# Rose-STL-Lab/spherical-dyffusion

Hardware: AMD Instinct MI355X
Metric: forecast-steps/sec (180x360, 63ch), 25-member ensemble DYffusion sampling, whole job (higher is better)
Workload: dtype f32 tensors; every GEMM-class kernel (1x1 convs, fused MLP, Legendre analysis/synthesis, dhconv) as 3-pass split-f16 MFMA with f32 accumulation; FFT / norms / pointwise in f32 (statistics f64); 1 GPU; 25-member ensemble x horizon-6 DYffusion sampling pass (6 forecaster + 10 interpolator SFNO forwards, dropout stream on, AR feedback), 180x360, 63 state + 2 forcing channels, embed 256, 8 blocks; horizon=6, relayed_members=0, parallelism=members of one initial condition sharded over GPUs, no data-path collective

## Files before the change

### spherical-dyffusion_amd/csrc/fft360.hip

```cpp
#include "common.h"
#include "fft.h"

namespace {

typedef float c2 __attribute__((ext_vector_type(2)));

constexpr int NH = 180;
constexpr int NLON = 360;
constexpr int ROWS = 16;
constexpr int NT = 256;
constexpr int P = 200;
constexpr int Q4 = NLON / 4;
constexpr int MIT = 3;
#ifndef SDY_FFT_MINB_F
#define SDY_FFT_MINB_F 4
#endif
#ifndef SDY_FFT_MINB_I
#define SDY_FFT_MINB_I 4
#endif
#ifndef SDY_FFT_KPW
#define SDY_FFT_KPW 1
#endif
constexpr int MINB_F = SDY_FFT_MINB_F, MINB_I = SDY_FFT_MINB_I;

template <int SG>
__device__ __forceinline__ c2 mul_i(c2 a) {
  return SG > 0 ? c2{-a.y, a.x} : c2{a.y, -a.x};
}
__device__ __forceinline__ c2 cmul(c2 a, c2 w) { return a.xx * w + a.yy * c2{-w.y, w.x}; }
__device__ __forceinline__ c2 cmul_conj(c2 a, c2 w) { return a.xx * c2{w.x, -w.y} + a.yy * c2{w.y, w.x}; }

template <int SG>
__device__ __forceinline__ void dft3(c2& v0, c2& v1, c2& v2) {
  const float sn = 0.86602540378443864676f;
  const c2 a = v1 + v2, b = v1 - v2;
  const c2 m = v0 - 0.5f * a;
  const c2 t = mul_i<SG>(sn * b);
  v0 = v0 + a;
  v1 = m + t;
  v2 = m - t;
}
template <int SG>
__device__ __forceinline__ void dft4(c2& v0, c2& v1, c2& v2, c2& v3) {
  const c2 t0 = v0 + v2, t1 = v0 - v2, t2 = v1 + v3, t3 = mul_i<SG>(v1 - v3);
  v0 = t0 + t2;
  v1 = t1 + t3;
  v2 = t0 - t2;
  v3 = t1 - t3;
}
template <int SG>
__device__ __forceinline__ void dft5(c2& v0, c2& v1, c2& v2, c2& v3, c2& v4) {
  const float c1 = 0.30901699437494742410f, c2_ = -0.80901699437494742410f;
  const float s1 = 0.95105651629515357212f, s2 = 0.58778525229247312917f;
  const c2 a1 = v1 + v4, a2 = v2 + v3, b1 = v1 - v4, b2 = v2 - v3;
  const c2 r1 = v0 + c1 * a1 + c2_ * a2;
  const c2 r2 = v0 + c2_ * a1 + c1 * a2;
  const c2 i1 = mul_i<SG>(s1 * b1 + s2 * b2);
  const c2 i2 = mul_i<SG>(s2 * b1 - s1 * b2);
  v0 = v0 + a1 + a2;
  v1 = r1 + i1;
  v4 = r1 - i1;
  v2 = r2 + i2;
  v3 = r2 - i2;
}
template <int R, int SG>
__device__ __forceinline__ void dft_small(c2* t) {
  if constexpr (R == 3) dft3<SG>(t[0], t[1], t[2]);
  if constexpr (R == 4) dft4<SG>(t[0], t[1], t[2], t[3]);
  if constexpr (R == 5) dft5<SG>(t[0], t[1], t[2], t[3], t[4]);
}

template <int N1, int N2>
__host__ __device__ constexpr int pfa_slot(int k) { return (N2 * (k % N1) + N1 * (k % N2)) % (N1 * N2); }
template <int N1, int N2, int SG>
__device__ __forceinline__ void pfa(c2* v) {
  constexpr int N = N1 * N2;
#pragma unroll
  for (int n2 = 0; n2 < N2; ++n2) {
    c2 t[N1];
#pragma unroll
    for (int n1 = 0; n1 < N1; ++n1) t[n1] = v[(N2 * n1 + N1 * n2) % N];
    dft_small<N1, SG>(t);
#pragma unroll
    for (int n1 = 0; n1 < N1; ++n1) v[(N2 * n1 + N1 * n2) % N] = t[n1];
  }
#pragma unroll
  for (int k1 = 0; k1 < N1; ++k1) {
    c2 u[N2];
#pragma unroll
    for (int n2 = 0; n2 < N2; ++n2) u[n2] = v[(N2 * k1 + N1 * n2) % N];
    dft_small<N2, SG>(u);
#pragma unroll
    for (int n2 = 0; n2 < N2; ++n2) v[(N2 * k1 + N1 * n2) % N] = u[n2];
  }
}

struct Lane {
  int wave, lane, t;
  c2* row;
};
__device__ __forceinline__ Lane lane_roles(c2* Z) {
  Lane L;
  L.wave = __builtin_amdgcn_readfirstlane(threadIdx.x >> 6);
  L.lane = threadIdx.x & 63;
  L.t = L.lane & 15;
  const int rl = L.lane >> 4;
  L.row = Z + (4 * L.wave + (rl & 1) * 2 + (rl >> 1)) * P;
  return L;
}

constexpr int TWN = 12 * 16;
__device__ __forceinline__ void fill_twiddles(const SdyFftDesc& f, c2* TW) {
  if (threadIdx.x < TWN) {
    const int k1 = threadIdx.x >> 4, a = threadIdx.x & 15;
    TW[threadIdx.x] = reinterpret_cast<const c2*>(f.tw)[a < 15 ? a * k1 : 0];
  }
}

template <int SG, bool NYQ_COPY>
__device__ __forceinline__ void pass_b(const Lane& L) {
  __builtin_amdgcn_wave_barrier();
  if (L.t < 12) {
    c2 u[15];
    const c2* src = L.row + 15 * L.t;
#pragma unroll
    for (int a = 0; a < 15; ++a) u[a] = src[a];
    pfa<3, 5, SG>(u);
    __builtin_amdgcn_wave_barrier();
    c2* dst = L.row + L.t;
#pragma unroll
    for (int k2 = 0; k2 < 15; ++k2) dst[12 * k2] = u[pfa_slot<3, 5>(k2)];
    if (NYQ_COPY && L.t == 0) dst[NH] = u[pfa_slot<3, 5>(0)];
  }
  __builtin_amdgcn_wave_barrier();
}
template <int SG>
__device__ __forceinline__ void pass_a_tail(const Lane& L, c2* v, const c2* TW) {
  pfa<3, 4, SG>(v);
  c2* dst = L.row + L.t;
  const c2* tw = TW + L.t;
  dst[0] = v[pfa_slot<3, 4>(0)];
#pragma unroll
  for (int k1 = 1; k1 < 12; ++k1) {
    const c2 y = v[pfa_slot<3, 4>(k1)];
    dst[15 * k1] = SG < 0 ? cmul(y, tw[16 * k1]) : cmul_conj(y, tw[16 * k1]);
  }
}

constexpr int TAIL = Q4 - 64;

#ifndef SDY_FFT_GROUP
#define SDY_FFT_GROUP 4
#endif
struct WgId {
  int x, y, z;
};
__device__ __forceinline__ WgId wg_id(int nx, int ny) {
  const unsigned total = gridDim.x, L = blockIdx.x;
  const unsigned xcd = L % 8u, slot = L / 8u;
  const unsigned id = xcd * (total / 8u) + min(xcd, total % 8u) + slot;
  WgId w;
#if SDY_FFT_GROUP > 0
  if (nx % SDY_FFT_GROUP == 0) {
    const unsigned G = SDY_FFT_GROUP;
    w.x = (int)(G * ((id / (G * ny)) % ((unsigned)nx / G)) + id % G);
    w.y = (int)((id / G) % (unsigned)ny);
    w.z = (int)(id / ((unsigned)nx * ny));
    return w;
  }
#endif
  w.x = id % nx;
  w.y = (id / nx) % ny;
  w.z = id / (nx * ny);
  return w;
}

template <int KPW>
__global__ __launch_bounds__(NT, MINB_F) void rfft360_kernel(const SdyFftDesc f, const float* __restrict__ x,
                                                           const float* __restrict__ pa, const float* __restrict__ pd,
                                                           float* __restrict__ xn_out, float* __restrict__ Xf, int B,
                                                           int C, int K, int mtr, int ilv,
                                                           const int* __restrict__ mcut, const SdyImgMap xmap,
                                                           unsigned* flags, unsigned* head, int x_mod) {
  __shared__ __attribute__((aligned(16))) c2 Z[ROWS * P];
  __shared__ c2 TW[TWN];
  __shared__ c2 AD[ROWS];
  const Lane L = lane_roles(Z);
  const WgId id = wg_id(C / ROWS, (K + KPW - 1) / KPW);
  const int c0 = id.x * ROWS, b = id.z;
  const int bx = sdy_img(xmap, b);
  const int k_begin = id.y * KPW, k_end = min(K, k_begin + KPW);

  fill_twiddles(f, TW);
  if (threadIdx.x < ROWS) {
    const int s = threadIdx.x, ch = c0 + 4 * (s & 3) + (s >> 2);
    AD[s] = pa ? c2{pa[bx * C + ch], pd[bx * C + ch]} : c2{1.0f, 0.0f};
  }

  const int bsrc = x_mod > 0 ? bx % x_mod : bx;
  const float* xw = x + (((long)bsrc * C + c0 + L.wave) * K) * NLON + 4 * L.lane;
  float* xnw = xn_out ? xn_out + (((long)bx * C + c0 + L.wave) * K) * NLON + 4 * L.lane : nullptr;
  const long rstride = 4L * K * NLON;
  c2* zw = Z + 4 * L.wave * P + 2 * L.lane;
  const bool tail = L.lane < TAIL;

  const int c4 = threadIdx.x & 3, mg = threadIdx.x >> 2;
  const float scale = 6.28318530717958647692f / (float)NLON;
  c2 W[MIT];
#pragma unroll
  for (int it = 0; it < MIT; ++it) {
    const c2 w = reinterpret_cast<const c2*>(f.pw)[min(mg + 64 * it, NH)];
    W[it] = c2{w.y, -w.x} * (0.5f * scale);
  }
  const c2* za = Z + c4 * P + mg;
  const c2* zn01 = Z + c4 * P + (NH - 64 - mg);
  const c2* zn2 = Z + c4 * P + max(NH - 128 - mg, 0);
  const long mstride = (long)K * B * 2 * C;
  const int re_off = (ilv ? 2 * c0 : c0) + 4 * c4, im_off = ilv ? 16 : C;
  const long tile_base = (long)((b * (C / ROWS) + id.x) >> 1) * K * 64 + (id.x & 1) * 32 + 4 * c4;

  float amax = 0.0f;
  f32x4 regs[8];
  auto gload = [&](int k) {
#pragma unroll
    for (int r = 0; r < 4; ++r) {
      const float* src = xw + r * rstride + (long)k * NLON;
      regs[2 * r] = *reinterpret_cast<const f32x4*>(src);
      if (tail) regs[2 * r + 1] = *reinterpret_cast<const f32x4*>(src + 256);
    }
  };
  gload(k_begin);
  __syncthreads();

  for (int k = k_begin; k < k_end; ++k) {
#pragma unroll
    for (int r = 0; r < 4; ++r) {
      const c2 ad = AD[4 * L.wave + r];
      const f32x4 v0 = regs[2 * r] * ad.x + ad.y, v1 = regs[2 * r + 1] * ad.x + ad.y;
      if (xnw) {
        float* dst = xnw + r * rstride + (long)k * NLON;
        *reinterpret_cast<f32x4*>(dst) = v0;
        if (tail) *reinterpret_cast<f32x4*>(dst + 256) = v1;
      }
      *reinterpret_cast<f32x4*>(zw + r * P) = v0;
      if (tail) *reinterpret_cast<f32x4*>(zw + r * P + 128) = v1;
    }
    if (k + 1 < k_end) gload(k + 1);
    __builtin_amdgcn_wave_barrier();

    if (L.t < 15) {
      c2 v[12];
      const c2* src = L.row + L.t;
#pragma unroll
      for (int bb = 0; bb < 12; ++bb) v[bb] = src[15 * bb];
      pass_a_tail<-1>(L, v, TW);
    }
    pass_b<-1, true>(L);
    __syncthreads();

    float* Xk = ilv == 2 ? Xf + tile_base + (long)k * 64 : Xf + ((long)k * B + b) * 2 * C + re_off;
    const int mlive = mcut ? min(mtr, mcut[k]) : mtr;
#pragma unroll
    for (int it = 0; it < MIT; ++it) {
      const int m = mg + 64 * it;
      if (m < mlive) {
        f32x4 vr, vi;
#pragma unroll
        for (int j = 0; j < 4; ++j) {
          const c2 A = za[64 * it + 4 * j * P];
          const c2 Bv = it < 2 ? zn01[64 * (1 - it) + 4 * j * P] : zn2[4 * j * P];
          const c2 S = c2{A.x + Bv.x, A.y - Bv.y}, D = c2{A.x - Bv.x, A.y + Bv.y};
          const c2 X = (0.5f * scale) * S + cmul(D, W[it]);
          vr[j] = X.x;
          vi[j] = X.y;
          amax = __builtin_fmaxf(amax, __builtin_fmaxf(__builtin_fabsf(X.x), __builtin_fabsf(X.y)));
        }
        float* o = Xk + (long)m * mstride;
        SDY_STREAM_STORE(o, vr);
        SDY_STREAM_STORE(o + im_off, vi);
      }
    }
    __syncthreads();
  }
  sdy_flag_range(flags, amax * (2.0f * SDY_ACT_SX), head);
}

template <int KPW>
__global__ __launch_bounds__(NT, MINB_I) void irfft360_kernel(const SdyFftDesc f, const float* __restrict__ Yf,
                                                            const float* __restrict__ bias, float* __restrict__ y, int B,
                                                            int C, int K, int mtr, int ilv,
                                                            const int* __restrict__ mcut, float* __restrict__ zt,
                                                            long zt_bs, double* __restrict__ part) {
  __shared__ __attribute__((aligned(16))) c2 Z[ROWS * P];
  __shared__ c2 TW[TWN];
  __shared__ c2 PW[NH];
  __shared__ float BS[ROWS];
  const Lane L = lane_roles(Z);
  const WgId id = wg_id(C / ROWS, (K + KPW - 1) / KPW);
  const int c0 = id.x * ROWS, b = id.z;
  const int k_begin = id.y * KPW, k_end = min(K, k_begin + KPW);

  fill_twiddles(f, TW);
  if (threadIdx.x < NH) {
    const c2 w = reinterpret_cast<const c2*>(f.pw)[threadIdx.x];
    PW[threadIdx.x] = c2{w.x, -w.y};
  }
  if (threadIdx.x < ROWS) {
    const int s = threadIdx.x;
    BS[s] = bias ? bias[c0 + 4 * (s & 3) + (s >> 2)] : 0.0f;
  }

  const int c4 = threadIdx.x & 3, mg = threadIdx.x >> 2;
  const long mstride = (long)K * B * 2 * C;
  const int re_off = (ilv ? 2 * c0 : c0) + 4 * c4, im_off = ilv ? 16 : C;
  const long tile_base = (long)((b * (C / ROWS) + id.x) >> 1) * K * 64 + (id.x & 1) * 32 + 4 * c4;
  f32x4 rr[MIT], ri[MIT];
  auto gload = [&](int k) {
    const float* Yk = ilv == 2 ? Yf + tile_base + (long)k * 64 : Yf + ((long)k * B + b) * 2 * C + re_off;
    const int mlive = mcut ? min(mtr, mcut[k]) : mtr;
#pragma unroll
    for (int it = 0; it < MIT; ++it) {
      const int m = mg + 64 * it;
      f32x4 vr = {0.f, 0.f, 0.f, 0.f}, vi = {0.f, 0.f, 0.f, 0.f};
      if (m < mlive) {
        const float* o = Yk + (long)m * mstride;
        vr = *reinterpret_cast<const f32x4*>(o);
        vi = *reinterpret_cast<const f32x4*>(o + im_off);
      }
      if (m == 0 || m == NH) vi = f32x4{0.f, 0.f, 0.f, 0.f};
      rr[it] = vr;
      ri[it] = vi;
    }
  };

  float* yw = y + (((long)b * C + c0 + L.wave) * K) * NLON + 4 * L.lane;
  const long rstride = 4L * K * NLON;
  const c2* zw = Z + 4 * L.wave * P + 2 * L.lane;
  const bool tail = L.lane < TAIL;
  c2* zs = Z + c4 * P + mg;

  gload(k_begin);
  for (int k = k_begin; k < k_end; ++k) {
#pragma unroll
    for (int it = 0; it < MIT; ++it) {
      if (mg + 64 * it <= NH) {
#pragma unroll
        for (int j = 0; j < 4; ++j) zs[4 * j * P + 64 * it] = c2{rr[it][j], ri[it][j]};
      }
    }
    __syncthreads();
    if (k + 1 < k_end) gload(k + 1);

    if (L.t < 15) {
      c2 v[12];
      const c2* lo = L.row + L.t;
      const c2* hi = L.row + (15 - L.t);
      const c2* pw = PW + L.t;
#pragma unroll
      for (int bb = 0; bb < 12; ++bb) {
        const c2 A = lo[15 * bb], Bv = hi[15 * (11 - bb)], w = pw[15 * bb];
        const c2 S = c2{A.x + Bv.x, A.y - Bv.y}, Dm = c2{A.x - Bv.x, A.y + Bv.y};
        const c2 D = cmul(Dm, w);
        v[bb] = c2{S.x - D.y, S.y + D.x};
      }
      __builtin_amdgcn_wave_barrier();
      pass_a_tail<+1>(L, v, TW);
    }
    pass_b<+1, false>(L);

    if (zt) {
      float* ztb = zt + (long)b * zt_bs;
      const int px0 = k * NLON + 4 * L.lane, px1 = px0 + 256;
#pragma unroll
      for (int r = 0; r < 4; ++r) {
        const float bs = BS[4 * L.wave + r];
        const int ch = c0 + L.wave + 4 * r;
        f32x4 v = *reinterpret_cast<const f32x4*>(zw + r * P) + bs;
        v = f32x4{gelu_erf(v.x), gelu_erf(v.y), gelu_erf(v.z), gelu_erf(v.w)};
        SDY_STREAM_STORE(ztb + (long)(px0 >> 6) * (C * 64) + ch * 64 + (px0 & 63), v);
        float qs = sdy_quad_sum(v), qs2 = sdy_quad_sumsq(v);
        if (tail) {
          f32x4 u = *reinterpret_cast<const f32x4*>(zw + r * P + 128) + bs;
          u = f32x4{gelu_erf(u.x), gelu_erf(u.y), gelu_erf(u.z), gelu_erf(u.w)};
          SDY_STREAM_STORE(ztb + (long)(px1 >> 6) * (C * 64) + ch * 64 + (px1 & 63), u);
          qs += sdy_quad_sum(u);
          qs2 += sdy_quad_sumsq(u);
        }
        double ds = (double)row16_sum(qs), ds2 = (double)row16_sum(qs2);
        ds += __shfl_xor(ds, 16, 64);
        ds2 += __shfl_xor(ds2, 16, 64);
        ds += __shfl_xor(ds, 32, 64);
        ds2 += __shfl_xor(ds2, 32, 64);
        if (L.lane == 0) {
          double* slot = part + (((long)b * K + k) * C + ch) * 2;
          slot[0] = ds;
          slot[1] = ds2;
        }
      }
    } else {
#pragma unroll
    for (int r = 0; r < 4; ++r) {
      const float bs = BS[4 * L.wave + r];
      float* dst = yw + r * rstride + (long)k * NLON;
      SDY_STREAM_STORE(dst, *reinterpret_cast<const f32x4*>(zw + r * P) + bs);
      if (tail) SDY_STREAM_STORE(dst + 256, *reinterpret_cast<const f32x4*>(zw + r * P + 128) + bs);
    }
    }
    __syncthreads();
  }
}

}

int sdy_fft360_launch_fwd(const SdyFftDesc& f, const float* x, const float* a, const float* d, float* xn_out, float* Xf,
                          int B, int C, int K, int mtr, int ilv, const int* mcut, hipStream_t stream,
                          const unsigned char* x_rows, int x_mod) {
  if (f.n != NH || C % ROWS != 0 || mtr > NH + 1 || (long)ROWS * K * NLON >= (1L << 31)) return SDY_ERR_UNSUPPORTED;
  if (ilv == 2 && (C % (2 * ROWS) != 0 || ROWS != 16)) return SDY_ERR_UNSUPPORTED;
  constexpr int KPW = SDY_FFT_KPW;
  SdyImgMap xmap;
  SDY_TRY(sdy_img_map_fill(xmap, x_rows, B));
  dim3 grid((C / ROWS) * ((K + KPW - 1) / KPW) * B);
  unsigned *flags = nullptr, *head = nullptr;
  if (f.guard_f16) {
    SDY_TRY(sdy_flags_ptr(&flags));
    SDY_TRY(sdy_headroom_ptr(SDY_RANGE_LEG_ANALYSIS, &head));
  }
  hipLaunchKernelGGL((rfft360_kernel<KPW>), grid, dim3(NT), 0, stream, f, x, a, d, xn_out, Xf, B, C, K, mtr, ilv, mcut, xmap,
                     flags, head, x_mod);
  return sdy_launch_status();
}

int sdy_fft360_launch_inv(const SdyFftDesc& f, const float* Yf, const float* bias, float* y, int B, int C, int K,
                          int mtr, int ilv, const int* mcut, hipStream_t stream, float* zt, long zt_bs, double* part) {
  if (f.n != NH || C % ROWS != 0 || mtr > NH + 1 || (long)ROWS * K * NLON >= (1L << 31)) return SDY_ERR_UNSUPPORTED;
  if (ilv == 2 && (C % (2 * ROWS) != 0 || ROWS != 16)) return SDY_ERR_UNSUPPORTED;
  if ((zt == nullptr) != (part == nullptr) || (!zt && !y)) return SDY_ERR_ARG;
  constexpr int KPW = SDY_FFT_KPW;
  dim3 grid((C / ROWS) * ((K + KPW - 1) / KPW) * B);
  hipLaunchKernelGGL((irfft360_kernel<KPW>), grid, dim3(NT), 0, stream, f, Yf, bias, y, B, C, K, mtr, ilv, mcut, zt, zt_bs, part);
  return sdy_launch_status();
}
```

Baseline: 165.1 member-forecast-steps/s.

## Shrink inverse FFT LDS row pitch, raise its occupancy bound, add timing stamps

Splits the shared-memory row pitch into separate forward and inverse values and cuts the inverse kernel's pitch from 200 to 184 complex elements. This lowers its LDS footprint, and with launch_bounds min blocks raised from 4 to 6 more workgroups can be resident per CU. A static_assert keeps the pitch at 8 or 24 mod 32 to avoid bank conflicts. It also adds env-gated s_memtime instrumentation and occupancy query exports under SDY_STAMPS_ON. The tighter launch bound may force register spills in the inverse kernel.

```diff
diff --git a/spherical-dyffusion_amd/csrc/fft360.hip b/spherical-dyffusion_amd/csrc/fft360.hip
--- a/spherical-dyffusion_amd/csrc/fft360.hip
+++ b/spherical-dyffusion_amd/csrc/fft360.hip
@@ -1,3 +1,5 @@
+#include <cstdlib>
+
 #include "common.h"
 #include "fft.h"
 
@@ -9,14 +11,21 @@
 constexpr int NLON = 360;
 constexpr int ROWS = 16;
 constexpr int NT = 256;
-constexpr int P = 200;
+#ifndef SDY_FFT_PITCH_F
+#define SDY_FFT_PITCH_F 200
+#endif
+#ifndef SDY_FFT_PITCH_I
+#define SDY_FFT_PITCH_I 184
+#endif
+constexpr int PF = SDY_FFT_PITCH_F, PI = SDY_FFT_PITCH_I;
+static_assert(PF >= NH + 1 && (PF % 32 == 8 || PF % 32 == 24) && PI >= NH + 1 && (PI % 32 == 8 || PI % 32 == 24), "row pitch");
 constexpr int Q4 = NLON / 4;
 constexpr int MIT = 3;
 #ifndef SDY_FFT_MINB_F
 #define SDY_FFT_MINB_F 4
 #endif
 #ifndef SDY_FFT_MINB_I
-#define SDY_FFT_MINB_I 4
+#define SDY_FFT_MINB_I 6
 #endif
 #ifndef SDY_FFT_KPW
 #define SDY_FFT_KPW 1
@@ -99,6 +108,7 @@
   int wave, lane, t;
   c2* row;
 };
+template <int P>
 __device__ __forceinline__ Lane lane_roles(c2* Z) {
   Lane L;
   L.wave = __builtin_amdgcn_readfirstlane(threadIdx.x >> 6);
@@ -182,10 +192,11 @@
                                                            int C, int K, int mtr, int ilv,
                                                            const int* __restrict__ mcut, const SdyImgMap xmap,
                                                            unsigned* flags, unsigned* head, int x_mod) {
+  constexpr int P = PF;
   __shared__ __attribute__((aligned(16))) c2 Z[ROWS * P];
   __shared__ c2 TW[TWN];
   __shared__ c2 AD[ROWS];
-  const Lane L = lane_roles(Z);
+  const Lane L = lane_roles<P>(Z);
   const WgId id = wg_id(C / ROWS, (K + KPW - 1) / KPW);
   const int c0 = id.x * ROWS, b = id.z;
   const int bx = sdy_img(xmap, b);
@@ -290,15 +301,29 @@
                                                             const float* __restrict__ bias, float* __restrict__ y, int B,
                                                             int C, int K, int mtr, int ilv,
                                                             const int* __restrict__ mcut, float* __restrict__ zt,
-                                                            long zt_bs, double* __restrict__ part) {
+                                                            long zt_bs, double* __restrict__ part,
+                                                            unsigned long long* stamps) {
+  constexpr int P = PI;
   __shared__ __attribute__((aligned(16))) c2 Z[ROWS * P];
   __shared__ c2 TW[TWN];
   __shared__ c2 PW[NH];
   __shared__ float BS[ROWS];
-  const Lane L = lane_roles(Z);
+  const Lane L = lane_roles<P>(Z);
   const WgId id = wg_id(C / ROWS, (K + KPW - 1) / KPW);
   const int c0 = id.x * ROWS, b = id.z;
   const int k_begin = id.y * KPW, k_end = min(K, k_begin + KPW);
+
+  unsigned long long* st = nullptr;
+  unsigned long long t_stats = 0;
+  if (SDY_STAMPS_ON && stamps && threadIdx.x == 0) {
+    const unsigned q = gridDim.x / 4u;
+    for (unsigned i = 0; i < 4; ++i)
+      if (blockIdx.x == q * i + q / 2u + 5u) st = stamps + (zt ? 64 : 0) + 16 * i;
+  }
+  auto stamp = [&](int i) {
+    if (SDY_STAMPS_ON && st) st[i] = __builtin_amdgcn_s_memtime();
+  };
+  stamp(0);
 
   fill_twiddles(f, TW);
   if (threadIdx.x < NH) {
@@ -340,7 +365,12 @@
   c2* zs = Z + c4 * P + mg;
 
   gload(k_begin);
+  stamp(1);
   for (int k = k_begin; k < k_end; ++k) {
+    if (SDY_STAMPS_ON && stamps) {
+      asm volatile("s_waitcnt vmcnt(0)" ::: "memory");
+      stamp(2);
+    }
 #pragma unroll
     for (int it = 0; it < MIT; ++it) {
       if (mg + 64 * it <= NH) {
@@ -349,6 +379,7 @@
       }
     }
     __syncthreads();
+    stamp(3);
     if (k + 1 < k_end) gload(k + 1);
 
     if (L.t < 15) {
@@ -366,7 +397,9 @@
       __builtin_amdgcn_wave_barrier();
       pass_a_tail<+1>(L, v, TW);
     }
+    stamp(4);
     pass_b<+1, false>(L);
+    stamp(5);
 
     if (zt) {
       float* ztb = zt + (long)b * zt_bs;
@@ -386,6 +419,8 @@
           qs += sdy_quad_sum(u);
           qs2 += sdy_quad_sumsq(u);
         }
+        unsigned long long ts0 = 0;
+        if (SDY_STAMPS_ON && st) ts0 = __builtin_amdgcn_s_memtime();
         double ds = (double)row16_sum(qs), ds2 = (double)row16_sum(qs2);
         ds += __shfl_xor(ds, 16, 64);
         ds2 += __shfl_xor(ds2, 16, 64);
@@ -396,6 +431,7 @@
           slot[0] = ds;
           slot[1] = ds2;
         }
+        if (SDY_STAMPS_ON && st) t_stats += __builtin_amdgcn_s_memtime() - ts0;
       }
     } else {
 #pragma unroll
@@ -406,11 +442,34 @@
       if (tail) SDY_STREAM_STORE(dst + 256, *reinterpret_cast<const f32x4*>(zw + r * P + 128) + bs);
     }
     }
+    stamp(6);
+    if (SDY_STAMPS_ON && stamps) {
+      asm volatile("s_waitcnt vmcnt(0)" ::: "memory");
+      stamp(7);
+    }
     __syncthreads();
-  }
-}
-
-}
+    stamp(8);
+    if (SDY_STAMPS_ON && st) st[9] = t_stats;
+  }
+}
+
+}
+
+#if SDY_STAMPS_ON
+static unsigned long long* g_istamps = nullptr;
+SDY_DEBUG_EXPORT int sdy_irfft360_debug_stamps(unsigned long long* host128) {
+  if (!g_istamps || !host128) return SDY_ERR_STATE;
+  SDY_HIP_TRY(hipDeviceSynchronize());
+  SDY_HIP_TRY(hipMemcpy(host128, g_istamps, 128 * sizeof(unsigned long long), hipMemcpyDeviceToHost));
+  return SDY_OK;
+}
+SDY_DEBUG_EXPORT int sdy_fft360_debug_occupancy(int* out2) {
+  if (!out2) return SDY_ERR_ARG;
+  SDY_HIP_TRY(hipOccupancyMaxActiveBlocksPerMultiprocessor(&out2[0], rfft360_kernel<SDY_FFT_KPW>, NT, 0));
+  SDY_HIP_TRY(hipOccupancyMaxActiveBlocksPerMultiprocessor(&out2[1], irfft360_kernel<SDY_FFT_KPW>, NT, 0));
+  return SDY_OK;
+}
+#endif
 
 int sdy_fft360_launch_fwd(const SdyFftDesc& f, const float* x, const float* a, const float* d, float* xn_out, float* Xf,
                           int B, int C, int K, int mtr, int ilv, const int* mcut, hipStream_t stream,
@@ -438,6 +497,17 @@
   if ((zt == nullptr) != (part == nullptr) || (!zt && !y)) return SDY_ERR_ARG;
   constexpr int KPW = SDY_FFT_KPW;
   dim3 grid((C / ROWS) * ((K + KPW - 1) / KPW) * B);
-  hipLaunchKernelGGL((irfft360_kernel<KPW>), grid, dim3(NT), 0, stream, f, Yf, bias, y, B, C, K, mtr, ilv, mcut, zt, zt_bs, part);
+  unsigned long long* stamps = nullptr;
+#if SDY_STAMPS_ON
+  if (std::getenv("SDY_IRFFT_STAMPS")) {
+    if (!g_istamps) {
+      SDY_HIP_TRY(hipMalloc(&g_istamps, 128 * sizeof(unsigned long long)));
+      SDY_HIP_TRY(hipMemset(g_istamps, 0, 128 * sizeof(unsigned long long)));
+    }
+    stamps = g_istamps;
+  }
+#endif
+  hipLaunchKernelGGL((irfft360_kernel<KPW>), grid, dim3(NT), 0, stream, f, Yf, bias, y, B, C, K, mtr, ilv, mcut, zt, zt_bs, part,
+                     stamps);
   return sdy_launch_status();
 }
```

Result: no change. 165.4 member-forecast-steps/s, median of 6 (+0.2%).
